# fabiojbg/LLMApiGateway

Measured on AMD Instinct MI355X. Metric: req/sec @ fixed QPS, higher is better.
Workload: dtype bf16; 1 GPU; model=llama-3-8b, global_batch=256, seq_len=192, prompt_len=128, parallelism=dp1, mode=open-loop-poisson, sampling=greedy, kv_dtype=auto

## Files before the change

### llmapigateway_amd/ops/__init__.py

```python

from __future__ import annotations

import os
from typing import Optional, Tuple

_TUNE_BASE = os.path.join(os.path.dirname(os.path.abspath(__file__)), "tunableop_gfx950.csv")
if os.path.exists(_TUNE_BASE.replace(".csv", "0.csv")):
    os.environ.setdefault("PYTORCH_TUNABLEOP_ENABLED", "1")
    os.environ.setdefault("PYTORCH_TUNABLEOP_TUNING", "0")
    os.environ.setdefault("PYTORCH_TUNABLEOP_FILENAME", _TUNE_BASE)

import torch

if torch.version.hip and os.path.exists(_TUNE_BASE.replace(".csv", "0.csv")):
    try:
        import torch.cuda.tunable as _tunable

        _tunable.enable(True)
        if os.environ.get("PYTORCH_TUNABLEOP_TUNING") != "1":
            _tunable.tuning_enable(False)
            _tunable.set_filename(_TUNE_BASE, insert_device_ordinal=True)
            _tunable.read_file(_TUNE_BASE.replace(".csv", "0.csv"))
    except Exception:
        pass

from . import reference
from .reference import build_rope_cache

_C = None
_C_ERR: Optional[str] = None
try:
    import importlib

    _C = importlib.import_module("._C", __name__)
except ImportError as e:
    _C_ERR = str(e)


def have_native() -> bool:
    return _C is not None


def _native():
    if _C is None:
        raise RuntimeError(
            "llmapigateway_amd.ops._C (gfx950 HIP extension) is not built but a GPU tensor "
            "reached the ops layer. Build it with `python setup.py build_ext --inplace` "
            f"(import error: {_C_ERR})"
        )
    return _C


def rmsnorm(x: torch.Tensor, weight: torch.Tensor, eps: float = 1e-5) -> torch.Tensor:
    if x.is_cuda:
        out = torch.empty_like(x)
        _native().rmsnorm(out, x, weight, eps)
        return out
    return reference.rmsnorm(x, weight, eps)


def rmsnorm_residual(
    x: torch.Tensor, residual: torch.Tensor, weight: torch.Tensor, eps: float = 1e-5
) -> Tuple[torch.Tensor, torch.Tensor]:
    if x.is_cuda:
        out = torch.empty_like(x)
        _native().rmsnorm_residual(out, x, residual, weight, eps)
        return out, residual
    return reference.rmsnorm_residual(x, residual, weight, eps)


def rope_inplace(
    q: torch.Tensor, k: torch.Tensor, positions: torch.Tensor, cos_sin: torch.Tensor
) -> None:
    if q.is_cuda:
        _native().rope_inplace(q, k, positions, cos_sin)
        return
    reference.rope_inplace(q, k, positions, cos_sin)


def swiglu(x: torch.Tensor) -> torch.Tensor:
    if x.is_cuda:
        inter = x.shape[-1] // 2
        out = torch.empty(
            (*x.shape[:-1], inter), dtype=x.dtype, device=x.device
        )
        _native().swiglu(out, x)
        return out
    return reference.swiglu(x)


def rope_and_kv_write(
    q: torch.Tensor,
    k: torch.Tensor,
    v: torch.Tensor,
    k_cache: torch.Tensor,
    v_cache: torch.Tensor,
    positions: torch.Tensor,
    cos_sin: torch.Tensor,
    slot_mapping: torch.Tensor,
    k_scale: Optional[torch.Tensor] = None,
    v_scale: Optional[torch.Tensor] = None,
) -> None:
    if q.is_cuda:
        _native().rope_kv_write(
            q, k, v, k_cache, v_cache, positions, cos_sin, slot_mapping,
            k_scale, v_scale,
        )
        return
    reference.rope_inplace(q, k, positions, cos_sin)
    reference.kv_cache_write(k, v, k_cache, v_cache, slot_mapping, k_scale, v_scale)


def kv_cache_write(
    k: torch.Tensor,
    v: torch.Tensor,
    k_cache: torch.Tensor,
    v_cache: torch.Tensor,
    slot_mapping: torch.Tensor,
    k_scale: Optional[torch.Tensor] = None,
    v_scale: Optional[torch.Tensor] = None,
) -> None:
    if k.is_cuda:
        _native().kv_cache_write(k, v, k_cache, v_cache, slot_mapping, k_scale, v_scale)
        return
    reference.kv_cache_write(k, v, k_cache, v_cache, slot_mapping, k_scale, v_scale)


QTILE = 64


def build_prefill_tiles(seqlens, device) -> Tuple[torch.Tensor, torch.Tensor]:
    tile_seq, tile_off = [], []
    for i, L in enumerate(seqlens):
        for off in range(0, int(L), QTILE):
            tile_seq.append(i)
            tile_off.append(off)
    return (
        torch.tensor(tile_seq, dtype=torch.int32, device=device),
        torch.tensor(tile_off, dtype=torch.int32, device=device),
    )


def attention_prefill(
    q: torch.Tensor,
    k: torch.Tensor,
    v: torch.Tensor,
    cu_seqlens: torch.Tensor,
    max_seqlen: int,
    scale: Optional[float] = None,
    causal: bool = True,
    tile_seq: Optional[torch.Tensor] = None,
    tile_off: Optional[torch.Tensor] = None,
    k_cache: Optional[torch.Tensor] = None,
    v_cache: Optional[torch.Tensor] = None,
    block_tables: Optional[torch.Tensor] = None,
    cached_lens: Optional[torch.Tensor] = None,
    k_scale: Optional[torch.Tensor] = None,
    v_scale: Optional[torch.Tensor] = None,
) -> torch.Tensor:
    if scale is None:
        scale = float(q.shape[-1]) ** -0.5
    if q.is_cuda:
        if not causal:
            raise NotImplementedError("GPU prefill kernel is causal-only")
        if tile_seq is None or tile_off is None:
            cu = cu_seqlens.cpu().tolist()
            seqlens = [cu[i + 1] - cu[i] for i in range(len(cu) - 1)]
            tile_seq, tile_off = build_prefill_tiles(seqlens, q.device)
        out = torch.empty_like(q)
        _native().attention_prefill(
            out, q, k, v, cu_seqlens.int(), tile_seq, tile_off, float(scale),
            k_cache, v_cache, block_tables, cached_lens, k_scale, v_scale,
        )
        return out
    return reference.attention_prefill(
        q, k, v, cu_seqlens, scale, causal,
        k_cache=k_cache, v_cache=v_cache,
        block_tables=block_tables, cached_lens=cached_lens,
        k_scale=k_scale, v_scale=v_scale,
    )


_SPLIT_SPAN = 2048
_DECODE_VER = int(os.environ.get("LLMAPI_DECODE_VER", "2"))
_decode_ws: dict = {}
_decode_ws_retired: list = []


def _decode_scratch(device, n_acc: int, n_ml: int):
    ws = _decode_ws.get(device.index)
    if ws is None or ws[0].numel() < n_acc or ws[1].numel() < n_ml:
        if ws is not None:
            _decode_ws_retired.append(ws)
        ws = (
            torch.empty(n_acc, dtype=torch.float32, device=device),
            torch.empty(n_ml, dtype=torch.float32, device=device),
        )
        _decode_ws[device.index] = ws
    return ws


def attention_decode(
    q: torch.Tensor,
    k_cache: torch.Tensor,
    v_cache: torch.Tensor,
    block_tables: torch.Tensor,
    context_lens: torch.Tensor,
    scale: Optional[float] = None,
    k_scale: Optional[torch.Tensor] = None,
    v_scale: Optional[torch.Tensor] = None,
) -> torch.Tensor:
    if scale is None:
        scale = float(q.shape[-1]) ** -0.5
    if q.is_cuda:
        out = torch.empty_like(q)
        B, Hq = q.shape[0], q.shape[1]
        max_ctx = block_tables.shape[1] * k_cache.shape[2]
        nsplit = 1
        if B * k_cache.shape[1] < 192 and max_ctx > _SPLIT_SPAN:
            nsplit = min(8, -(-max_ctx // _SPLIT_SPAN))
        if nsplit > 1:
            pa, pm = _decode_scratch(
                q.device, B * Hq * nsplit * q.shape[2], B * Hq * nsplit * 2
            )
            _native().attention_decode(
                out, q, k_cache, v_cache, block_tables, context_lens,
                float(scale), pa, pm, nsplit, k_scale, v_scale, 1,
            )
        else:
            _native().attention_decode(
                out, q, k_cache, v_cache, block_tables, context_lens,
                float(scale), None, None, 1, k_scale, v_scale, _DECODE_VER,
            )
        return out
    return reference.attention_decode(
        q, k_cache, v_cache, block_tables, context_lens, scale,
        k_scale=k_scale, v_scale=v_scale,
    )


_SKINNY_MAX_M = int(os.environ.get("SKINNY_GEMM_MAX_M", "16"))
_SKINNY_MAX_N = 28672
_skinny_ws: dict = {}


def _skinny_nsk(N: int, K: int) -> int:
    tiles = N // 64
    nsk = max(1, -(-256 // tiles))
    nsk = min(nsk, max(1, (K // 32) // 8), 8)
    return nsk


_skinny_ws_retired: list = []


def _skinny_scratch(device, numel: int):
    ws = _skinny_ws.get(device.index)
    if ws is None or ws.numel() < numel:
        if ws is not None:
            _skinny_ws_retired.append(ws)
        ws = torch.empty(numel, dtype=torch.float32, device=device)
        _skinny_ws[device.index] = ws
    return ws


def swizzle_weight(w: torch.Tensor) -> torch.Tensor:
    N, K = w.shape
    assert K % 32 == 0 and N % 64 == 0
    return w.view(N, K // 32, 32).permute(1, 0, 2).contiguous()


def swizzle_weight_frag(w: torch.Tensor) -> torch.Tensor:
    N, K = w.shape
    assert K % 64 == 0 and N % 64 == 0
    return (
        w.view(N // 16, 16, K // 32, 4, 8)
        .permute(2, 0, 3, 1, 4)
        .reshape(K // 32, N // 16, 64, 8)
        .contiguous()
    )


def _m256_config(M: int, N: int, K: int) -> Optional[dict]:
    if M > 256:
        return None
    if N == 8192 and K % 64 == 0 and K >= 8192:
        if K > 8192:
            return {"nf": 8, "nsk": 4, "variant": 1, "pipe": 0}
        return {"nf": 8, "nsk": 4, "variant": 0, "pipe": 0}
    if N == 7168 and K <= 8192:
        return {"nf": 4, "nsk": 3, "variant": 0, "pipe": 4}
    if N > 4096:
        return None
    if K > 8192 and N % 128 == 0:
        return {"nf": 8, "nsk": 8, "variant": 0, "pipe": 0}
    if N < 2048:
        return None
    if K < 2048:
        return {"nf": 4, "nsk": 1, "variant": 1, "pipe": 0}
    tiles = N // 64
    nsk = max(1, min(-(-256 // tiles), (K // 64) // 2, 8))
    return {"nf": 4, "nsk": nsk, "variant": 0, "pipe": 4}


def _m256_nsk(N: int, K: int, nf: int) -> int:
    tiles = N // (16 * nf)
    if tiles >= 256:
        return 1
    nsk = -(-256 // tiles)
    return max(1, min(nsk, (K // 64) // 2, 8))


_SKINNY_SWZ_MAX_M = int(os.environ.get("SKINNY_GEMM_SWZ_MAX_M", "256"))


_M256_VARIANT = int(os.environ.get("LLMAPI_M256_VARIANT", "0"))


def gemm_m256(
    x: torch.Tensor, w_frag: torch.Tensor, nf: Optional[int] = None,
    nsk: Optional[int] = None, variant: Optional[int] = None,
    pipe: Optional[int] = None,
) -> torch.Tensor:
    M, K = x.shape
    N = w_frag.shape[1] * 16
    if nf is None:
        if N % 128 == 0 and M > 64:
            nf = 8
        else:
            nf = 8 if N // 64 >= 448 else 4
    if N % (16 * nf) != 0:
        nf = 4
    if nsk is None:
        nsk = _m256_nsk(N, K, nf)
    if variant is None:
        variant = _M256_VARIANT
    if pipe is None:
        pipe = 3 if (variant == 0 and nf == 8 and K % 32 == 0) else 0
    if variant == 0:
        if pipe in (2, 3) and nf != 8:
            pipe = 0
        if pipe in (1, 4, 5) and nf != 4:
            pipe = 0
    y = torch.empty((M, N), dtype=torch.bfloat16, device=x.device)
    ws = _skinny_scratch(x.device, nsk * M * N) if nsk > 1 else None
    _native().gemm_m256(y, x, w_frag, ws, nsk, nf, variant, pipe, 0)
    return y


def _reduce_norm_covers(N: int) -> bool:
    return N % 512 == 0 and 0 < N <= 8192


def gemm_m256_rmsnorm_residual(
    x: torch.Tensor, w_frag: torch.Tensor, residual: torch.Tensor,
    norm_w: torch.Tensor, eps: float, nf: int, nsk: int, variant: int = 0,
    pipe: int = 0,
) -> Tuple[torch.Tensor, torch.Tensor]:
    M, K = x.shape
    N = w_frag.shape[1] * 16
    if nsk < 2:
        raise ValueError("fused reduce+norm needs split-K slabs (nsk > 1)")
    out = torch.empty((M, N), dtype=torch.bfloat16, device=x.device)
    ws = _skinny_scratch(x.device, nsk * M * N)
    _native().gemm_m256(
        out, x, w_frag, ws, nsk, nf, variant, pipe, 0,
        residual, norm_w, float(eps), out,
    )
    return out, residual


def _m256_route(
    x: torch.Tensor, w: torch.Tensor, w_swz: Optional[torch.Tensor]
) -> Optional[dict]:
    M = x.shape[0]
    if not (
        x.is_cuda
        and x.dim() == 2
        and x.dtype == torch.bfloat16
        and w.dtype == torch.bfloat16
        and w.shape[0] % 64 == 0
        and w.shape[0] <= _SKINNY_MAX_N
        and w.shape[1] % 64 == 0
        and x.is_contiguous()
        and w.is_contiguous()
        and w_swz is not None
        and w_swz.dim() == 4
        and 8 < M <= 256
    ):
        return None
    return _m256_config(M, w.shape[0], w.shape[1])


def linear_rmsnorm_residual(
    x: torch.Tensor, w: torch.Tensor, w_swz: Optional[torch.Tensor],
    residual: torch.Tensor, norm_w: torch.Tensor, eps: float = 1e-5,
) -> Tuple[torch.Tensor, torch.Tensor]:
    if not x.is_cuda:
        return reference.linear_rmsnorm_residual(x, w, residual, norm_w, eps)
    if not os.environ.get("LLMAPI_NO_DECODE_FUSION"):
        cfg = _m256_route(x, w, w_swz)
        if (
            cfg is not None
            and cfg["nsk"] > 1
            and _reduce_norm_covers(w.shape[0])
            and residual.is_contiguous()
        ):
            return gemm_m256_rmsnorm_residual(
                x, w_swz, residual, norm_w, eps, **cfg
            )
    return rmsnorm_residual(linear(x, w, w_swz), residual, norm_w, eps)


def interleave_gate_up(w: torch.Tensor) -> torch.Tensor:
    two_i, K = w.shape
    assert two_i % 32 == 0
    return w.view(2, two_i // 32, 16, K).transpose(0, 1).reshape(two_i, K)


def gemm_m256_swiglu(
    x: torch.Tensor, w_frag: torch.Tensor, nf: int = 8, variant: int = 1,
    pipe: int = 0,
) -> torch.Tensor:
    M, K = x.shape
    N = w_frag.shape[1] * 16
    y = torch.empty((M, N // 2), dtype=torch.bfloat16, device=x.device)
    _native().gemm_m256(y, x, w_frag, None, 1, nf, variant, pipe, 1)
    return y


def _m256_swiglu_config(M: int, N: int, K: int) -> Optional[dict]:
    if os.environ.get("LLMAPI_NO_FUSED_SWIGLU"):
        return None
    if not (8 < M <= 256):
        return None
    if N == 28672 and K == 4096:
        if M <= 128:
            return {"nf": 8, "variant": 0, "pipe": 0}
        return {"nf": 8, "variant": 1, "pipe": 0}
    if N == 7168 and K == 4096:
        return {"nf": 4, "variant": 0, "pipe": 4}
    return None


def swiglu_linear(
    x: torch.Tensor, w: torch.Tensor,
    w_swz: Optional[torch.Tensor] = None,
    w_int: Optional[torch.Tensor] = None,
) -> torch.Tensor:
    if w_int is not None and x.dim() == 2:
        cfg = _m256_swiglu_config(x.shape[0], w_int.shape[1] * 16, x.shape[1])
        if cfg is not None:
            return gemm_m256_swiglu(x, w_int, **cfg)
    return swiglu(linear(x, w, w_swz))


def linear(
    x: torch.Tensor, w: torch.Tensor, w_swz: Optional[torch.Tensor] = None
) -> torch.Tensor:
    M = x.shape[0]
    if (
        x.is_cuda
        and x.dtype == torch.bfloat16
        and w.dtype == torch.bfloat16
        and 0 < M
        and w.shape[0] % 64 == 0
        and w.shape[0] <= _SKINNY_MAX_N
        and w.shape[1] % 32 == 0
        and x.is_contiguous()
        and w.is_contiguous()
    ):
        N, K = w.shape
        if (
            w_swz is not None
            and w_swz.dim() == 4
            and 8 < M <= 256
            and K % 64 == 0
        ):
            cfg = _m256_config(M, N, K)
            if cfg is not None:
                return gemm_m256(x, w_swz, **cfg)
            return torch.nn.functional.linear(x, w)
        if w_swz is not None and w_swz.dim() == 3 and M <= _SKINNY_SWZ_MAX_M:
            y = torch.empty((M, N), dtype=torch.bfloat16, device=x.device)
            nsk = _skinny_nsk(N, K)
            ws = _skinny_scratch(x.device, nsk * M * N) if nsk > 1 else None
            _native().gemm_skinny(y, x, w_swz, ws, nsk, True)
            return y
        if M <= _SKINNY_MAX_M:
            y = torch.empty((M, N), dtype=torch.bfloat16, device=x.device)
            nsk = _skinny_nsk(N, K)
            ws = _skinny_scratch(x.device, nsk * M * N) if nsk > 1 else None
            _native().gemm_skinny(y, x, w, ws, nsk, False)
            return y
    return torch.nn.functional.linear(x, w)


def topk_topp_filter(
    logits: torch.Tensor, topp: torch.Tensor, topk: torch.Tensor
) -> torch.Tensor:
    if logits.is_cuda:
        _native().topk_topp_filter(logits, topp, topk)
        return logits
    return reference.topk_topp_filter(logits, topp, topk)


def sample(
    logits: torch.Tensor,
    temperature: torch.Tensor,
    noise: Optional[torch.Tensor] = None,
) -> torch.Tensor:
    if logits.is_cuda:
        out = torch.empty(logits.shape[0], dtype=torch.long, device=logits.device)
        _native().sample(out, logits, temperature, noise)
        return out
    return reference.sample(logits, temperature, noise)


__all__ = [
    "have_native",
    "build_rope_cache",
    "rmsnorm",
    "rmsnorm_residual",
    "rope_inplace",
    "rope_and_kv_write",
    "swiglu",
    "kv_cache_write",
    "linear",
    "gemm_m256",
    "gemm_m256_rmsnorm_residual",
    "linear_rmsnorm_residual",
    "swizzle_weight",
    "swizzle_weight_frag",
    "attention_prefill",
    "attention_decode",
    "sample",
    "topk_topp_filter",
    "reference",
]
```

### llmapigateway_amd/ops/csrc/attention_decode.hip

```cpp

#include "common.h"

#define MAX_G 8
#define NWAVES 4
#define DECODE_D 128
#define SPLIT_SPAN 2048

template <int G, bool SPLIT, bool FP8>
__launch_bounds__(NWAVES* WAVE_SIZE)
__global__ void attention_decode_kernel(
    bf16* __restrict__ out,
    const bf16* __restrict__ q,
    const void* __restrict__ k_cache,
    const void* __restrict__ v_cache,
    const float* __restrict__ k_scale,
    const float* __restrict__ v_scale,
    const int* __restrict__ block_tables,
    const int* __restrict__ context_lens,
    float scale,
    int Hq,
    int Hkv,
    int block_size,
    int max_blocks,
    int64_t q_stride,
    float* __restrict__ part_acc,
    float* __restrict__ part_ml,
    int nsplit) {
    const int seq = blockIdx.x;
    const int kvh = blockIdx.y;
    const int split = SPLIT ? blockIdx.z : 0;
    const int D = DECODE_D;
    const int L = context_lens[seq];
    if (L <= 0) return;
    const int span0 = SPLIT ? split * SPLIT_SPAN : 0;
    if (SPLIT && span0 >= L) {
        const int lane0 = threadIdx.x & (WAVE_SIZE - 1);
        if (threadIdx.x < WAVE_SIZE) {
#pragma unroll
            for (int g = 0; g < G; ++g) {
                const size_t pb =
                    (((size_t)seq * Hq + kvh * G + g) * nsplit + split);
                if (lane0 < 2) part_ml[pb * 2 + lane0] = lane0 == 0 ? -INFINITY : 0.f;
                for (int d = lane0; d < D; d += WAVE_SIZE) part_acc[pb * D + d] = 0.f;
            }
        }
        return;
    }
    const int span1 = SPLIT ? min(L, span0 + SPLIT_SPAN) : L;

    const int tid = threadIdx.x;
    const int lane = tid & (WAVE_SIZE - 1);
    const int wave = tid >> 6;

    __shared__ float q_lds[G][DECODE_D];
    __shared__ float p_lds[NWAVES][G][WAVE_SIZE];
    __shared__ float m_lds[NWAVES][G];
    __shared__ float l_lds[NWAVES][G];
    __shared__ float acc_lds[NWAVES][G][DECODE_D];
    __shared__ int bt_lds[1024];

    for (int i = tid; i < G * D; i += blockDim.x) {
        const int g = i / D, d = i % D;
        q_lds[g][d] =
            bf2f(q[(size_t)seq * q_stride + (size_t)(kvh * G + g) * D + d]) * scale;
    }
    const int nblocks = (L + block_size - 1) / block_size;
    for (int i = tid; i < nblocks && i < 1024; i += blockDim.x)
        bt_lds[i] = block_tables[(size_t)seq * max_blocks + i];
    __syncthreads();
    const int* __restrict__ bt_global = block_tables + (size_t)seq * max_blocks;
#define BT(idx) ((idx) < 1024 ? bt_lds[(idx)] : bt_global[(idx)])

    float m[G], l[G], acc[G][4];
#pragma unroll
    for (int g = 0; g < G; ++g) {
        m[g] = -INFINITY;
        l[g] = 0.f;
#pragma unroll
        for (int d = 0; d < 4; ++d) acc[g][d] = 0.f;
    }

    const int c0 = span0 / WAVE_SIZE;
    const int nchunks = (span1 + WAVE_SIZE - 1) / WAVE_SIZE;
    for (int c = c0 + wave; c < nchunks; c += NWAVES) {
        const int pos = c * WAVE_SIZE + lane;
        const bool valid = pos < span1;

        float s[G];
#pragma unroll
        for (int g = 0; g < G; ++g) s[g] = valid ? 0.f : -INFINITY;
        if (valid) {
            const int kblock = BT(pos / block_size);
            const int koff = pos % block_size;
            const size_t krow_i = ((size_t)kblock * Hkv + kvh) * block_size + koff;
#pragma unroll 4
            for (int i = 0; i < D / 8; ++i) {
                float kf[8];
                if (FP8) {
                    const uint2 kq = reinterpret_cast<const uint2*>(
                        (const unsigned char*)k_cache + krow_i * D)[i];
                    fp8x4_to_f32(kq.x, kf[0], kf[1], kf[2], kf[3]);
                    fp8x4_to_f32(kq.y, kf[4], kf[5], kf[6], kf[7]);
                } else {
                    const uint4 kv8 = reinterpret_cast<const uint4*>(
                        (const bf16*)k_cache + krow_i * D)[i];
                    unpack2(kv8.x, kf[0], kf[1]);
                    unpack2(kv8.y, kf[2], kf[3]);
                    unpack2(kv8.z, kf[4], kf[5]);
                    unpack2(kv8.w, kf[6], kf[7]);
                }
#pragma unroll
                for (int g = 0; g < G; ++g) {
                    const float4 qa = *reinterpret_cast<const float4*>(&q_lds[g][i * 8]);
                    const float4 qb = *reinterpret_cast<const float4*>(&q_lds[g][i * 8 + 4]);
                    s[g] = fmaf(qa.x, kf[0], s[g]);
                    s[g] = fmaf(qa.y, kf[1], s[g]);
                    s[g] = fmaf(qa.z, kf[2], s[g]);
                    s[g] = fmaf(qa.w, kf[3], s[g]);
                    s[g] = fmaf(qb.x, kf[4], s[g]);
                    s[g] = fmaf(qb.y, kf[5], s[g]);
                    s[g] = fmaf(qb.z, kf[6], s[g]);
                    s[g] = fmaf(qb.w, kf[7], s[g]);
                }
            }
            if (FP8) {
                const float ksc = k_scale[krow_i];
#pragma unroll
                for (int g = 0; g < G; ++g) s[g] *= ksc;
            }
        }

#pragma unroll
        for (int g = 0; g < G; ++g) {
            const float cmax = wave_reduce_max(s[g]);
            const float m_new = fmaxf(m[g], cmax);
            float p = 0.f;
            if (valid && m_new != -INFINITY) p = __expf(s[g] - m_new);
            const float factor = (m[g] == -INFINITY) ? 0.f : __expf(m[g] - m_new);
            const float csum = wave_reduce_sum(p);
            l[g] = l[g] * factor + csum;
#pragma unroll
            for (int d = 0; d < 4; ++d) acc[g][d] *= factor;
            m[g] = m_new;
            p_lds[wave][g][lane] = p;
        }

        const int dbase = (lane & 31) * 4;
        const int khalf = lane >> 5;
#pragma unroll 2
        for (int j = 0; j < WAVE_SIZE; j += 8) {
            uint2 vp[4];
            uint32_t vp8[4];
            float vsc[4];
#pragma unroll
            for (int u = 0; u < 4; ++u) {
                const int pos = min(c * WAVE_SIZE + j + 2 * u + khalf, span1 - 1);
                const int vb = BT(pos / block_size);
                const int vo = pos % block_size;
                const size_t vrow_i = ((size_t)vb * Hkv + kvh) * block_size + vo;
                if (FP8) {
                    vp8[u] = *reinterpret_cast<const uint32_t*>(
                        (const unsigned char*)v_cache + vrow_i * D + dbase);
                    vsc[u] = v_scale[vrow_i];
                } else {
                    vp[u] = *reinterpret_cast<const uint2*>(
                        (const bf16*)v_cache + vrow_i * D + dbase);
                }
            }
#pragma unroll
            for (int u = 0; u < 4; ++u) {
                float v0, v1, v2, v3;
                if (FP8) {
                    fp8x4_to_f32(vp8[u], v0, v1, v2, v3);
                } else {
                    unpack2(vp[u].x, v0, v1);
                    unpack2(vp[u].y, v2, v3);
                }
                const int key = j + 2 * u + khalf;
#pragma unroll
                for (int g = 0; g < G; ++g) {
                    const float pj = p_lds[wave][g][key] * (FP8 ? vsc[u] : 1.f);
                    acc[g][0] = fmaf(pj, v0, acc[g][0]);
                    acc[g][1] = fmaf(pj, v1, acc[g][1]);
                    acc[g][2] = fmaf(pj, v2, acc[g][2]);
                    acc[g][3] = fmaf(pj, v3, acc[g][3]);
                }
            }
        }
    }

#pragma unroll
    for (int g = 0; g < G; ++g)
#pragma unroll
        for (int d = 0; d < 4; ++d) acc[g][d] += __shfl_xor(acc[g][d], 32, WAVE_SIZE);

#pragma unroll
    for (int g = 0; g < G; ++g) {
        if (lane == 0) {
            m_lds[wave][g] = m[g];
            l_lds[wave][g] = l[g];
        }
        if (lane < 32) {
#pragma unroll
            for (int d = 0; d < 4; ++d)
                acc_lds[wave][g][(lane & 31) * 4 + d] = acc[g][d];
        }
    }
    __syncthreads();

    if (wave == 0) {
#pragma unroll
        for (int g = 0; g < G; ++g) {
            float gm = -INFINITY;
#pragma unroll
            for (int w = 0; w < NWAVES; ++w) gm = fmaxf(gm, m_lds[w][g]);
            float gl = 0.f;
            float f[NWAVES];
#pragma unroll
            for (int w = 0; w < NWAVES; ++w) {
                f[w] = (m_lds[w][g] == -INFINITY) ? 0.f : __expf(m_lds[w][g] - gm);
                gl += f[w] * l_lds[w][g];
            }
            float o0 = 0.f, o1 = 0.f;
#pragma unroll
            for (int w = 0; w < NWAVES; ++w) {
                o0 += f[w] * acc_lds[w][g][2 * lane];
                o1 += f[w] * acc_lds[w][g][2 * lane + 1];
            }
            if (SPLIT) {
                const size_t pb =
                    (((size_t)seq * Hq + kvh * G + g) * nsplit + split);
                part_acc[pb * DECODE_D + 2 * lane] = o0;
                part_acc[pb * DECODE_D + 2 * lane + 1] = o1;
                if (lane == 0) {
                    part_ml[pb * 2] = gm;
                    part_ml[pb * 2 + 1] = gl;
                }
            } else {
                const float inv_l = (gl > 0.f) ? 1.f / gl : 0.f;
                reinterpret_cast<uint32_t*>(
                    out + (size_t)seq * Hq * DECODE_D +
                    (size_t)(kvh * G + g) * DECODE_D)[lane] =
                    pack2(o0 * inv_l, o1 * inv_l);
            }
        }
    }
}

typedef __attribute__((__vector_size__(8 * sizeof(short)))) short bf16x8_d;


template <int G, bool SPLIT, bool FP8>
__launch_bounds__(NWAVES* WAVE_SIZE)
__global__ void attention_decode_v2_kernel(
    bf16* __restrict__ out,
    const bf16* __restrict__ q,
    const void* __restrict__ k_cache,
    const void* __restrict__ v_cache,
    const float* __restrict__ k_scale,
    const float* __restrict__ v_scale,
    const int* __restrict__ block_tables,
    const int* __restrict__ context_lens,
    float scale,
    int Hq,
    int Hkv,
    int block_size,
    int max_blocks,
    int64_t q_stride,
    float* __restrict__ part_acc,
    float* __restrict__ part_ml,
    int nsplit) {
    const int seq = blockIdx.x;
    const int kvh = blockIdx.y;
    const int split = SPLIT ? blockIdx.z : 0;
    const int D = DECODE_D;
    const int L = context_lens[seq];
    if (L <= 0) return;
    const int span0 = SPLIT ? split * SPLIT_SPAN : 0;
    const int tid = threadIdx.x;
    const int lane = tid & (WAVE_SIZE - 1);
    const int wave = tid >> 6;
    constexpr int HPW = (G + NWAVES - 1) / NWAVES;
    if (SPLIT && span0 >= L) {
#pragma unroll
        for (int hh = 0; hh < HPW; ++hh) {
            const int g = wave + hh * NWAVES;
            if (g >= G) break;
            const size_t pb = (((size_t)seq * Hq + kvh * G + g) * nsplit + split);
            if (lane < 2) part_ml[pb * 2 + lane] = lane == 0 ? -INFINITY : 0.f;
            for (int d = lane; d < D; d += WAVE_SIZE) part_acc[pb * D + d] = 0.f;
        }
        return;
    }
    const int span1 = SPLIT ? min(L, span0 + SPLIT_SPAN) : L;

    __shared__ float q_lds[G][DECODE_D];
    __shared__ bf16 k_lds[WAVE_SIZE][DECODE_D];
    __shared__ bf16 v_lds[WAVE_SIZE][DECODE_D];
    __shared__ float p_lds[G][WAVE_SIZE];
    __shared__ int bt_lds[1024];

    for (int i = tid; i < G * D; i += blockDim.x) {
        const int g = i / D, d = i % D;
        q_lds[g][d] =
            bf2f(q[(size_t)seq * q_stride + (size_t)(kvh * G + g) * D + d]) * scale;
    }
    const int nblocks = (L + block_size - 1) / block_size;
    for (int i = tid; i < nblocks && i < 1024; i += blockDim.x)
        bt_lds[i] = block_tables[(size_t)seq * max_blocks + i];
    __syncthreads();
    const int* __restrict__ bt_global = block_tables + (size_t)seq * max_blocks;
#define BT2(idx) ((idx) < 1024 ? bt_lds[(idx)] : bt_global[(idx)])

    float m[HPW], l[HPW], acc[HPW][4];
#pragma unroll
    for (int h = 0; h < HPW; ++h) {
        m[h] = -INFINITY;
        l[h] = 0.f;
#pragma unroll
        for (int d = 0; d < 4; ++d) acc[h][d] = 0.f;
    }

    const int c0 = span0 / WAVE_SIZE;
    const int nchunks = (span1 + WAVE_SIZE - 1) / WAVE_SIZE;
    for (int c = c0; c < nchunks; ++c) {
        __syncthreads();
        for (int pass = 0; pass < 4; ++pass) {
            const int key = (pass << 4) | (tid >> 4);
            const int chunk = tid & 15;
            const int pos = c * WAVE_SIZE + key;
            const int cpos = min(pos, span1 - 1);
            const int blk = BT2(cpos / block_size);
            const size_t row =
                ((size_t)blk * Hkv + kvh) * block_size + cpos % block_size;
            const int kchunk = chunk ^ (key & 15);
            if (FP8) {
                const uint2 kq = reinterpret_cast<const uint2*>(
                    (const unsigned char*)k_cache + row * D)[chunk];
                const uint2 vq = reinterpret_cast<const uint2*>(
                    (const unsigned char*)v_cache + row * D)[chunk];
                const float ksc = k_scale[row], vsc = v_scale[row];
                float kf[8], vf[8];
                fp8x4_to_f32(kq.x, kf[0], kf[1], kf[2], kf[3]);
                fp8x4_to_f32(kq.y, kf[4], kf[5], kf[6], kf[7]);
                fp8x4_to_f32(vq.x, vf[0], vf[1], vf[2], vf[3]);
                fp8x4_to_f32(vq.y, vf[4], vf[5], vf[6], vf[7]);
                uint2 kw, vw;
                kw.x = pack2_trunc(kf[0] * ksc, kf[1] * ksc);
                kw.y = pack2_trunc(kf[2] * ksc, kf[3] * ksc);
                uint2 kw2;
                kw2.x = pack2_trunc(kf[4] * ksc, kf[5] * ksc);
                kw2.y = pack2_trunc(kf[6] * ksc, kf[7] * ksc);
                vw.x = pack2_trunc(vf[0] * vsc, vf[1] * vsc);
                vw.y = pack2_trunc(vf[2] * vsc, vf[3] * vsc);
                uint2 vw2;
                vw2.x = pack2_trunc(vf[4] * vsc, vf[5] * vsc);
                vw2.y = pack2_trunc(vf[6] * vsc, vf[7] * vsc);
                uint4 kq4 = {kw.x, kw.y, kw2.x, kw2.y};
                uint4 vq4 = {vw.x, vw.y, vw2.x, vw2.y};
                *reinterpret_cast<uint4*>(&k_lds[key][kchunk * 8]) = kq4;
                *reinterpret_cast<uint4*>(&v_lds[key][chunk * 8]) = vq4;
            } else {
                *reinterpret_cast<uint4*>(&k_lds[key][kchunk * 8]) =
                    reinterpret_cast<const uint4*>((const bf16*)k_cache + row * D)[chunk];
                *reinterpret_cast<uint4*>(&v_lds[key][chunk * 8]) =
                    reinterpret_cast<const uint4*>((const bf16*)v_cache + row * D)[chunk];
            }
        }
        __syncthreads();

        const int pos = c * WAVE_SIZE + lane;
        const bool valid = pos < span1;
#pragma unroll
        for (int hh = 0; hh < HPW; ++hh) {
            const int g = wave + hh * NWAVES;
            if (g >= G) break;
            float sg = valid ? 0.f : -INFINITY;
            if (valid) {
#pragma unroll 4
                for (int i = 0; i < D / 8; ++i) {
                    const bf16x8_d kv8 = *reinterpret_cast<const bf16x8_d*>(
                        &k_lds[lane][(i ^ (lane & 15)) * 8]);
                    const uint4 kvu = *reinterpret_cast<const uint4*>(&kv8);
                    float kf[8];
                    unpack2(kvu.x, kf[0], kf[1]);
                    unpack2(kvu.y, kf[2], kf[3]);
                    unpack2(kvu.z, kf[4], kf[5]);
                    unpack2(kvu.w, kf[6], kf[7]);
                    const float4 qa = *reinterpret_cast<const float4*>(&q_lds[g][i * 8]);
                    const float4 qb = *reinterpret_cast<const float4*>(&q_lds[g][i * 8 + 4]);
                    sg = fmaf(qa.x, kf[0], sg);
                    sg = fmaf(qa.y, kf[1], sg);
                    sg = fmaf(qa.z, kf[2], sg);
                    sg = fmaf(qa.w, kf[3], sg);
                    sg = fmaf(qb.x, kf[4], sg);
                    sg = fmaf(qb.y, kf[5], sg);
                    sg = fmaf(qb.z, kf[6], sg);
                    sg = fmaf(qb.w, kf[7], sg);
                }
            }
            const float cmax = wave_reduce_max(sg);
            const float m_new = fmaxf(m[hh], cmax);
            float pv = 0.f;
            if (valid && m_new != -INFINITY) pv = __expf(sg - m_new);
            const float factor = (m[hh] == -INFINITY) ? 0.f : __expf(m[hh] - m_new);
            const float csum = wave_reduce_sum(pv);
            l[hh] = l[hh] * factor + csum;
#pragma unroll
            for (int d = 0; d < 4; ++d) acc[hh][d] *= factor;
            m[hh] = m_new;
            p_lds[g][lane] = pv;
        }

        const int dbase = (lane & 31) * 4;
        const int khalf = lane >> 5;
#pragma unroll
        for (int hh = 0; hh < HPW; ++hh) {
            const int g = wave + hh * NWAVES;
            if (g >= G) break;
#pragma unroll 4
            for (int j = 0; j < WAVE_SIZE; j += 2) {
                const int key = j + khalf;
                const float pj = p_lds[g][key];
                float v0, v1, v2, v3;
                const uint2 vv = *reinterpret_cast<const uint2*>(&v_lds[key][dbase]);
                unpack2(vv.x, v0, v1);
                unpack2(vv.y, v2, v3);
                acc[hh][0] = fmaf(pj, v0, acc[hh][0]);
                acc[hh][1] = fmaf(pj, v1, acc[hh][1]);
                acc[hh][2] = fmaf(pj, v2, acc[hh][2]);
                acc[hh][3] = fmaf(pj, v3, acc[hh][3]);
            }
        }
    }

#pragma unroll
    for (int hh = 0; hh < HPW; ++hh) {
        const int g = wave + hh * NWAVES;
        if (g >= G) break;
#pragma unroll
        for (int d = 0; d < 4; ++d) acc[hh][d] += __shfl_xor(acc[hh][d], 32, WAVE_SIZE);
        if (lane < 32) {
            if (SPLIT) {
                const size_t pb = (((size_t)seq * Hq + kvh * G + g) * nsplit + split);
#pragma unroll
                for (int d = 0; d < 4; ++d)
                    part_acc[pb * DECODE_D + (lane & 31) * 4 + d] = acc[hh][d];
                if (lane == 0) {
                    part_ml[pb * 2] = m[hh];
                    part_ml[pb * 2 + 1] = l[hh];
                }
            } else {
                const float inv_l = (l[hh] > 0.f) ? 1.f / l[hh] : 0.f;
                uint2 o2;
                o2.x = pack2(acc[hh][0] * inv_l, acc[hh][1] * inv_l);
                o2.y = pack2(acc[hh][2] * inv_l, acc[hh][3] * inv_l);
                *reinterpret_cast<uint2*>(
                    out + (size_t)seq * Hq * DECODE_D +
                    (size_t)(kvh * G + g) * DECODE_D + (lane & 31) * 4) = o2;
            }
        }
    }
}

template <int G, bool SPLIT, bool FP8>
__launch_bounds__(NWAVES* WAVE_SIZE)
__global__ void attention_decode_v3_kernel(
    bf16* __restrict__ out,
    const bf16* __restrict__ q,
    const void* __restrict__ k_cache,
    const void* __restrict__ v_cache,
    const float* __restrict__ k_scale,
    const float* __restrict__ v_scale,
    const int* __restrict__ block_tables,
    const int* __restrict__ context_lens,
    float scale,
    int Hq,
    int Hkv,
    int block_size,
    int max_blocks,
    int64_t q_stride,
    float* __restrict__ part_acc,
    float* __restrict__ part_ml,
    int nsplit) {
    const int seq = blockIdx.x;
    const int kvh = blockIdx.y;
    const int split = SPLIT ? blockIdx.z : 0;
    const int D = DECODE_D;
    const int L = context_lens[seq];
    if (L <= 0) return;
    const int span0 = SPLIT ? split * SPLIT_SPAN : 0;
    const int tid = threadIdx.x;
    const int lane = tid & (WAVE_SIZE - 1);
    const int wave = tid >> 6;
    constexpr int HPW = (G + NWAVES - 1) / NWAVES;
    if (SPLIT && span0 >= L) {
#pragma unroll
        for (int hh = 0; hh < HPW; ++hh) {
            const int g = wave + hh * NWAVES;
            if (g >= G) break;
            const size_t pb = (((size_t)seq * Hq + kvh * G + g) * nsplit + split);
            if (lane < 2) part_ml[pb * 2 + lane] = lane == 0 ? -INFINITY : 0.f;
            for (int d = lane; d < D; d += WAVE_SIZE) part_acc[pb * D + d] = 0.f;
        }
        return;
    }
    const int span1 = SPLIT ? min(L, span0 + SPLIT_SPAN) : L;

    __shared__ float q_lds[G][DECODE_D];
    __shared__ bf16 k_lds[WAVE_SIZE][DECODE_D];
    __shared__ float p_lds[G][WAVE_SIZE];
    __shared__ int bt_lds[1024];

    for (int i = tid; i < G * D; i += blockDim.x) {
        const int g = i / D, d = i % D;
        q_lds[g][d] =
            bf2f(q[(size_t)seq * q_stride + (size_t)(kvh * G + g) * D + d]) * scale;
    }
    const int nblocks = (L + block_size - 1) / block_size;
    for (int i = tid; i < nblocks && i < 1024; i += blockDim.x)
        bt_lds[i] = block_tables[(size_t)seq * max_blocks + i];
    __syncthreads();
    const int* __restrict__ bt_global = block_tables + (size_t)seq * max_blocks;
#define BT2(idx) ((idx) < 1024 ? bt_lds[(idx)] : bt_global[(idx)])

    float m[HPW], l[HPW], acc[HPW][4];
#pragma unroll
    for (int h = 0; h < HPW; ++h) {
        m[h] = -INFINITY;
        l[h] = 0.f;
#pragma unroll
        for (int d = 0; d < 4; ++d) acc[h][d] = 0.f;
    }

    const int c0 = span0 / WAVE_SIZE;
    const int nchunks = (span1 + WAVE_SIZE - 1) / WAVE_SIZE;
    for (int c = c0; c < nchunks; ++c) {
        __syncthreads();
        for (int pass = 0; pass < 4; ++pass) {
            const int key = (pass << 4) | (tid >> 4);
            const int chunk = tid & 15;
            const int pos = c * WAVE_SIZE + key;
            const int cpos = min(pos, span1 - 1);
            const int blk = BT2(cpos / block_size);
            const size_t row =
                ((size_t)blk * Hkv + kvh) * block_size + cpos % block_size;
            const int kchunk = chunk ^ (key & 15);
            if (FP8) {
                const uint2 kq = reinterpret_cast<const uint2*>(
                    (const unsigned char*)k_cache + row * D)[chunk];
                const float ksc = k_scale[row];
                float kf[8];
                fp8x4_to_f32(kq.x, kf[0], kf[1], kf[2], kf[3]);
                fp8x4_to_f32(kq.y, kf[4], kf[5], kf[6], kf[7]);
                uint4 kq4;
                kq4.x = pack2_trunc(kf[0] * ksc, kf[1] * ksc);
                kq4.y = pack2_trunc(kf[2] * ksc, kf[3] * ksc);
                kq4.z = pack2_trunc(kf[4] * ksc, kf[5] * ksc);
                kq4.w = pack2_trunc(kf[6] * ksc, kf[7] * ksc);
                *reinterpret_cast<uint4*>(&k_lds[key][kchunk * 8]) = kq4;
            } else {
                *reinterpret_cast<uint4*>(&k_lds[key][kchunk * 8]) =
                    reinterpret_cast<const uint4*>((const bf16*)k_cache + row * D)[chunk];
            }
        }
        __syncthreads();

        const int pos = c * WAVE_SIZE + lane;
        const bool valid = pos < span1;
#pragma unroll
        for (int hh = 0; hh < HPW; ++hh) {
            const int g = wave + hh * NWAVES;
            if (g >= G) break;
            float sg = valid ? 0.f : -INFINITY;
            if (valid) {
#pragma unroll 4
                for (int i = 0; i < D / 8; ++i) {
                    const bf16x8_d kv8 = *reinterpret_cast<const bf16x8_d*>(
                        &k_lds[lane][(i ^ (lane & 15)) * 8]);
                    const uint4 kvu = *reinterpret_cast<const uint4*>(&kv8);
                    float kf[8];
                    unpack2(kvu.x, kf[0], kf[1]);
                    unpack2(kvu.y, kf[2], kf[3]);
                    unpack2(kvu.z, kf[4], kf[5]);
                    unpack2(kvu.w, kf[6], kf[7]);
                    const float4 qa = *reinterpret_cast<const float4*>(&q_lds[g][i * 8]);
                    const float4 qb = *reinterpret_cast<const float4*>(&q_lds[g][i * 8 + 4]);
                    sg = fmaf(qa.x, kf[0], sg);
                    sg = fmaf(qa.y, kf[1], sg);
                    sg = fmaf(qa.z, kf[2], sg);
                    sg = fmaf(qa.w, kf[3], sg);
                    sg = fmaf(qb.x, kf[4], sg);
                    sg = fmaf(qb.y, kf[5], sg);
                    sg = fmaf(qb.z, kf[6], sg);
                    sg = fmaf(qb.w, kf[7], sg);
                }
            }
            const float cmax = wave_reduce_max(sg);
            const float m_new = fmaxf(m[hh], cmax);
            float pv = 0.f;
            if (valid && m_new != -INFINITY) pv = __expf(sg - m_new);
            const float factor = (m[hh] == -INFINITY) ? 0.f : __expf(m[hh] - m_new);
            const float csum = wave_reduce_sum(pv);
            l[hh] = l[hh] * factor + csum;
#pragma unroll
            for (int d = 0; d < 4; ++d) acc[hh][d] *= factor;
            m[hh] = m_new;
            p_lds[g][lane] = pv;
        }

        const int dbase = (lane & 31) * 4;
        const int khalf = lane >> 5;
#pragma unroll 2
        for (int j = 0; j < WAVE_SIZE; j += 8) {
            uint2 vp[4];
            uint32_t vp8[4];
            float vsc4[4];
#pragma unroll
            for (int u = 0; u < 4; ++u) {
                const int pos2 = min(c * WAVE_SIZE + j + 2 * u + khalf, span1 - 1);
                const int vb = BT2(pos2 / block_size);
                const int vo = pos2 % block_size;
                const size_t vrow = ((size_t)vb * Hkv + kvh) * block_size + vo;
                if (FP8) {
                    vp8[u] = *reinterpret_cast<const uint32_t*>(
                        (const unsigned char*)v_cache + vrow * D + dbase);
                    vsc4[u] = v_scale[vrow];
                } else {
                    vp[u] = *reinterpret_cast<const uint2*>(
                        (const bf16*)v_cache + vrow * D + dbase);
                }
            }
#pragma unroll
            for (int u = 0; u < 4; ++u) {
                float v0, v1, v2, v3;
                if (FP8) {
                    fp8x4_to_f32(vp8[u], v0, v1, v2, v3);
                } else {
                    unpack2(vp[u].x, v0, v1);
                    unpack2(vp[u].y, v2, v3);
                }
                const int key = j + 2 * u + khalf;
#pragma unroll
                for (int hh = 0; hh < HPW; ++hh) {
                    const int g = wave + hh * NWAVES;
                    if (g >= G) break;
                    const float pj = p_lds[g][key] * (FP8 ? vsc4[u] : 1.f);
                    acc[hh][0] = fmaf(pj, v0, acc[hh][0]);
                    acc[hh][1] = fmaf(pj, v1, acc[hh][1]);
                    acc[hh][2] = fmaf(pj, v2, acc[hh][2]);
                    acc[hh][3] = fmaf(pj, v3, acc[hh][3]);
                }
            }
        }
    }

#pragma unroll
    for (int hh = 0; hh < HPW; ++hh) {
        const int g = wave + hh * NWAVES;
        if (g >= G) break;
#pragma unroll
        for (int d = 0; d < 4; ++d) acc[hh][d] += __shfl_xor(acc[hh][d], 32, WAVE_SIZE);
        if (lane < 32) {
            if (SPLIT) {
                const size_t pb = (((size_t)seq * Hq + kvh * G + g) * nsplit + split);
#pragma unroll
                for (int d = 0; d < 4; ++d)
                    part_acc[pb * DECODE_D + (lane & 31) * 4 + d] = acc[hh][d];
                if (lane == 0) {
                    part_ml[pb * 2] = m[hh];
                    part_ml[pb * 2 + 1] = l[hh];
                }
            } else {
                const float inv_l = (l[hh] > 0.f) ? 1.f / l[hh] : 0.f;
                uint2 o2;
                o2.x = pack2(acc[hh][0] * inv_l, acc[hh][1] * inv_l);
                o2.y = pack2(acc[hh][2] * inv_l, acc[hh][3] * inv_l);
                *reinterpret_cast<uint2*>(
                    out + (size_t)seq * Hq * DECODE_D +
                    (size_t)(kvh * G + g) * DECODE_D + (lane & 31) * 4) = o2;
            }
        }
    }
}


__global__ void decode_combine_kernel(
    bf16* __restrict__ out,
    const float* __restrict__ part_acc,
    const float* __restrict__ part_ml,
    int nsplit) {
    const int bh = blockIdx.x;
    const int lane = threadIdx.x;
    const size_t base = (size_t)bh * nsplit;
    float gm = -INFINITY;
    for (int z = 0; z < nsplit; ++z) gm = fmaxf(gm, part_ml[(base + z) * 2]);
    float gl = 0.f, o0 = 0.f, o1 = 0.f;
    for (int z = 0; z < nsplit; ++z) {
        const float mz = part_ml[(base + z) * 2];
        const float f = (mz == -INFINITY) ? 0.f : __expf(mz - gm);
        gl += f * part_ml[(base + z) * 2 + 1];
        o0 += f * part_acc[(base + z) * DECODE_D + 2 * lane];
        o1 += f * part_acc[(base + z) * DECODE_D + 2 * lane + 1];
    }
    const float inv_l = (gl > 0.f) ? 1.f / gl : 0.f;
    reinterpret_cast<uint32_t*>(out + (size_t)bh * DECODE_D)[lane] =
        pack2(o0 * inv_l, o1 * inv_l);
}

extern "C" hipError_t launch_attention_decode(
    void* out, const void* q, const void* k_cache, const void* v_cache,
    const float* k_scale, const float* v_scale,
    const int* block_tables, const int* context_lens, float scale, int B,
    int Hq, int Hkv, int block_size, int max_blocks, int D, int64_t q_stride,
    float* part_acc, float* part_ml, int nsplit, int version,
    hipStream_t stream) {
    if (D != DECODE_D) return hipErrorNotSupported;
    if (Hq % Hkv != 0) return hipErrorInvalidValue;
    if (nsplit > 1 && (part_acc == nullptr || part_ml == nullptr))
        return hipErrorInvalidValue;
    const int G = Hq / Hkv;
    const bool fp8 = k_scale != nullptr;
    dim3 grid(B, Hkv, nsplit > 1 ? nsplit : 1);
    dim3 block(NWAVES * WAVE_SIZE);
#define LAUNCH_G3(GV, SPLIT, FP8V)                                             \
    do {                                                                       \
        if (version == 2)                                                      \
            attention_decode_v2_kernel<GV, SPLIT, FP8V>                        \
                <<<grid, block, 0, stream>>>(                                  \
                    (bf16*)out, (const bf16*)q, k_cache, v_cache, k_scale,     \
                    v_scale, block_tables, context_lens, scale, Hq, Hkv,       \
                    block_size, max_blocks, q_stride, part_acc, part_ml,       \
                    nsplit);                                                   \
        else                                                                   \
            attention_decode_kernel<GV, SPLIT, FP8V>                           \
                <<<grid, block, 0, stream>>>(                                  \
                    (bf16*)out, (const bf16*)q, k_cache, v_cache, k_scale,     \
                    v_scale, block_tables, context_lens, scale, Hq, Hkv,       \
                    block_size, max_blocks, q_stride, part_acc, part_ml,       \
                    nsplit);                                                   \
    } while (0)
#define LAUNCH_G2(GV, SPLIT)                                                   \
    do {                                                                       \
        if (fp8) LAUNCH_G3(GV, SPLIT, true); else LAUNCH_G3(GV, SPLIT, false);\
    } while (0)
#define LAUNCH_G(GV)                                                           \
    do {                                                                       \
        if (nsplit > 1) LAUNCH_G2(GV, true); else LAUNCH_G2(GV, false);        \
    } while (0)
    switch (G) {
        case 1: LAUNCH_G(1); break;
        case 2: LAUNCH_G(2); break;
        case 3: LAUNCH_G(3); break;
        case 4: LAUNCH_G(4); break;
        case 5: LAUNCH_G(5); break;
        case 6: LAUNCH_G(6); break;
        case 7: LAUNCH_G(7); break;
        case 8: LAUNCH_G(8); break;
        default: return hipErrorInvalidValue;
    }
#undef LAUNCH_G
#undef LAUNCH_G2
#undef LAUNCH_G3
    if (nsplit > 1) {
        decode_combine_kernel<<<dim3(B * Hq), dim3(WAVE_SIZE), 0, stream>>>(
            (bf16*)out, part_acc, part_ml, nsplit);
    }
    HIP_CHECK_LAST();
    return hipSuccess;
}
```

Baseline: 189.9 req/s.

## Add register-prefetched decode attention kernel staging K and V through LDS

Adds a v4 decode attention kernel and makes it the default instead of v2. Each iteration prefetches the next chunk's K and V rows into registers while the current chunk is being computed. V is now staged in LDS with coalesced loads, replacing strided per-lane global reads. The Q load is issued before the early-exit check, and PV accumulation is bounded to the valid keys. The costs are more registers, an extra LDS buffer for V, and a new code path that may lower occupancy.

Result: no change. 189.3 req/s (-0.3%).

```diff
diff --git a/llmapigateway_amd/ops/__init__.py b/llmapigateway_amd/ops/__init__.py
--- a/llmapigateway_amd/ops/__init__.py
+++ b/llmapigateway_amd/ops/__init__.py
@@ -182,7 +182,7 @@
 
 
 _SPLIT_SPAN = 2048
-_DECODE_VER = int(os.environ.get("LLMAPI_DECODE_VER", "2"))
+_DECODE_VER = int(os.environ.get("LLMAPI_DECODE_VER", "4"))
 _decode_ws: dict = {}
 _decode_ws_retired: list = []
 
diff --git a/llmapigateway_amd/ops/csrc/attention_decode.hip b/llmapigateway_amd/ops/csrc/attention_decode.hip
--- a/llmapigateway_amd/ops/csrc/attention_decode.hip
+++ b/llmapigateway_amd/ops/csrc/attention_decode.hip
@@ -463,9 +463,102 @@
     }
 }
 
+
+template <bool FP8>
+struct DecodeStage;
+template <>
+struct DecodeStage<false> {
+    uint4 k[4], v[4];
+};
+template <>
+struct DecodeStage<true> {
+    uint2 k[4], v[4];
+    float ks[4], vs[4];
+};
+
+template <bool FP8, typename BTF>
+__device__ __forceinline__ void decode_stage_load(
+    DecodeStage<FP8>& st, int c, int span1, int tid, int Hkv, int kvh,
+    int block_size, const void* __restrict__ k_cache,
+    const void* __restrict__ v_cache, const float* __restrict__ k_scale,
+    const float* __restrict__ v_scale, BTF bt) {
+    const int D = DECODE_D;
+    const int chunk = tid & 15;
+    int blk[4];
+#pragma unroll
+    for (int pass = 0; pass < 4; ++pass) {
+        const int pos = c * WAVE_SIZE + ((pass << 4) | (tid >> 4));
+        blk[pass] = bt(min(pos, span1 - 1) / block_size);
+    }
+    asm volatile("" ::"v"(blk[0]), "v"(blk[1]), "v"(blk[2]), "v"(blk[3]));
+#pragma unroll
+    for (int pass = 0; pass < 4; ++pass) {
+        const int pos = c * WAVE_SIZE + ((pass << 4) | (tid >> 4));
+        const size_t row =
+            ((size_t)blk[pass] * Hkv + kvh) * block_size + pos % block_size;
+        if constexpr (FP8) {
+            st.k[pass] = make_uint2(0u, 0u);
+            st.v[pass] = make_uint2(0u, 0u);
+            st.ks[pass] = 0.f;
+            st.vs[pass] = 0.f;
+            if (pos < span1) {
+                st.k[pass] = reinterpret_cast<const uint2*>(
+                    (const unsigned char*)k_cache + row * D)[chunk];
+                st.v[pass] = reinterpret_cast<const uint2*>(
+                    (const unsigned char*)v_cache + row * D)[chunk];
+                st.ks[pass] = k_scale[row];
+                st.vs[pass] = v_scale[row];
+            }
+        } else {
+            st.k[pass] = make_uint4(0u, 0u, 0u, 0u);
+            st.v[pass] = make_uint4(0u, 0u, 0u, 0u);
+            if (pos < span1) {
+                st.k[pass] = reinterpret_cast<const uint4*>(
+                    (const bf16*)k_cache + row * D)[chunk];
+                st.v[pass] = reinterpret_cast<const uint4*>(
+                    (const bf16*)v_cache + row * D)[chunk];
+            }
+        }
+    }
+}
+
+template <bool FP8>
+__device__ __forceinline__ void decode_stage_write(
+    const DecodeStage<FP8>& st, int tid, bf16 (*k_lds)[DECODE_D],
+    bf16 (*v_lds)[DECODE_D]) {
+    const int chunk = tid & 15;
+#pragma unroll
+    for (int pass = 0; pass < 4; ++pass) {
+        const int key = (pass << 4) | (tid >> 4);
+        const int kchunk = chunk ^ (key & 15);
+        if constexpr (FP8) {
+            const float ksc = st.ks[pass], vsc = st.vs[pass];
+            float kf[8], vf[8];
+            fp8x4_to_f32(st.k[pass].x, kf[0], kf[1], kf[2], kf[3]);
+            fp8x4_to_f32(st.k[pass].y, kf[4], kf[5], kf[6], kf[7]);
+            fp8x4_to_f32(st.v[pass].x, vf[0], vf[1], vf[2], vf[3]);
+            fp8x4_to_f32(st.v[pass].y, vf[4], vf[5], vf[6], vf[7]);
+            uint4 kq4, vq4;
+            kq4.x = pack2_trunc(kf[0] * ksc, kf[1] * ksc);
+            kq4.y = pack2_trunc(kf[2] * ksc, kf[3] * ksc);
+            kq4.z = pack2_trunc(kf[4] * ksc, kf[5] * ksc);
+            kq4.w = pack2_trunc(kf[6] * ksc, kf[7] * ksc);
+            vq4.x = pack2_trunc(vf[0] * vsc, vf[1] * vsc);
+            vq4.y = pack2_trunc(vf[2] * vsc, vf[3] * vsc);
+            vq4.z = pack2_trunc(vf[4] * vsc, vf[5] * vsc);
+            vq4.w = pack2_trunc(vf[6] * vsc, vf[7] * vsc);
+            *reinterpret_cast<uint4*>(&k_lds[key][kchunk * 8]) = kq4;
+            *reinterpret_cast<uint4*>(&v_lds[key][chunk * 8]) = vq4;
+        } else {
+            *reinterpret_cast<uint4*>(&k_lds[key][kchunk * 8]) = st.k[pass];
+            *reinterpret_cast<uint4*>(&v_lds[key][chunk * 8]) = st.v[pass];
+        }
+    }
+}
+
 template <int G, bool SPLIT, bool FP8>
 __launch_bounds__(NWAVES* WAVE_SIZE)
-__global__ void attention_decode_v3_kernel(
+__global__ void attention_decode_v4_kernel(
     bf16* __restrict__ out,
     const bf16* __restrict__ q,
     const void* __restrict__ k_cache,
@@ -487,10 +580,17 @@
     const int kvh = blockIdx.y;
     const int split = SPLIT ? blockIdx.z : 0;
     const int D = DECODE_D;
+    const int tid = threadIdx.x;
+    constexpr int QN = (G * DECODE_D + NWAVES * WAVE_SIZE - 1) / (NWAVES * WAVE_SIZE);
+    bf16 qv[QN];
+#pragma unroll
+    for (int u = 0; u < QN; ++u) {
+        const int i = min(tid + u * NWAVES * WAVE_SIZE, G * D - 1);
+        qv[u] = q[(size_t)seq * q_stride + (size_t)(kvh * G) * D + i];
+    }
     const int L = context_lens[seq];
     if (L <= 0) return;
     const int span0 = SPLIT ? split * SPLIT_SPAN : 0;
-    const int tid = threadIdx.x;
     const int lane = tid & (WAVE_SIZE - 1);
     const int wave = tid >> 6;
     constexpr int HPW = (G + NWAVES - 1) / NWAVES;
@@ -509,20 +609,30 @@
 
     __shared__ float q_lds[G][DECODE_D];
     __shared__ bf16 k_lds[WAVE_SIZE][DECODE_D];
+    __shared__ bf16 v_lds[WAVE_SIZE][DECODE_D];
     __shared__ float p_lds[G][WAVE_SIZE];
     __shared__ int bt_lds[1024];
 
-    for (int i = tid; i < G * D; i += blockDim.x) {
-        const int g = i / D, d = i % D;
-        q_lds[g][d] =
-            bf2f(q[(size_t)seq * q_stride + (size_t)(kvh * G + g) * D + d]) * scale;
-    }
+    const int c0 = span0 / WAVE_SIZE;
+    const int nchunks = (span1 + WAVE_SIZE - 1) / WAVE_SIZE;
+    const int* __restrict__ bt_global = block_tables + (size_t)seq * max_blocks;
+
     const int nblocks = (L + block_size - 1) / block_size;
-    for (int i = tid; i < nblocks && i < 1024; i += blockDim.x)
-        bt_lds[i] = block_tables[(size_t)seq * max_blocks + i];
-    __syncthreads();
-    const int* __restrict__ bt_global = block_tables + (size_t)seq * max_blocks;
-#define BT2(idx) ((idx) < 1024 ? bt_lds[(idx)] : bt_global[(idx)])
+    const int bt_first = bt_global[min(tid, nblocks - 1)];
+    DecodeStage<FP8> st;
+    decode_stage_load<FP8>(st, c0, span1, tid, Hkv, kvh, block_size, k_cache,
+                           v_cache, k_scale, v_scale,
+                           [&](int idx) { return bt_global[idx]; });
+
+#pragma unroll
+    for (int u = 0; u < QN; ++u) {
+        const int i = tid + u * NWAVES * WAVE_SIZE;
+        if (i < G * D) q_lds[i / D][i % D] = bf2f(qv[u]) * scale;
+    }
+    if (tid < nblocks) bt_lds[tid] = bt_first;
+    for (int i = tid + NWAVES * WAVE_SIZE; i < nblocks && i < 1024;
+         i += NWAVES * WAVE_SIZE)
+        bt_lds[i] = bt_global[i];
 
     float m[HPW], l[HPW], acc[HPW][4];
 #pragma unroll
@@ -533,38 +643,22 @@
         for (int d = 0; d < 4; ++d) acc[h][d] = 0.f;
     }
 
-    const int c0 = span0 / WAVE_SIZE;
-    const int nchunks = (span1 + WAVE_SIZE - 1) / WAVE_SIZE;
     for (int c = c0; c < nchunks; ++c) {
+        if (c != c0) __syncthreads();
+        decode_stage_write<FP8>(st, tid, k_lds, v_lds);
         __syncthreads();
-        for (int pass = 0; pass < 4; ++pass) {
-            const int key = (pass << 4) | (tid >> 4);
-            const int chunk = tid & 15;
-            const int pos = c * WAVE_SIZE + key;
-            const int cpos = min(pos, span1 - 1);
-            const int blk = BT2(cpos / block_size);
-            const size_t row =
-                ((size_t)blk * Hkv + kvh) * block_size + cpos % block_size;
-            const int kchunk = chunk ^ (key & 15);
-            if (FP8) {
-                const uint2 kq = reinterpret_cast<const uint2*>(
-                    (const unsigned char*)k_cache + row * D)[chunk];
-                const float ksc = k_scale[row];
-                float kf[8];
-                fp8x4_to_f32(kq.x, kf[0], kf[1], kf[2], kf[3]);
-                fp8x4_to_f32(kq.y, kf[4], kf[5], kf[6], kf[7]);
-                uint4 kq4;
-                kq4.x = pack2_trunc(kf[0] * ksc, kf[1] * ksc);
-                kq4.y = pack2_trunc(kf[2] * ksc, kf[3] * ksc);
-                kq4.z = pack2_trunc(kf[4] * ksc, kf[5] * ksc);
-                kq4.w = pack2_trunc(kf[6] * ksc, kf[7] * ksc);
-                *reinterpret_cast<uint4*>(&k_lds[key][kchunk * 8]) = kq4;
-            } else {
-                *reinterpret_cast<uint4*>(&k_lds[key][kchunk * 8]) =
-                    reinterpret_cast<const uint4*>((const bf16*)k_cache + row * D)[chunk];
-            }
-        }
-        __syncthreads();
+        if (c + 1 < nchunks) {
+            if (((c + 1) * WAVE_SIZE + WAVE_SIZE - 1) / block_size < 1024)
+                decode_stage_load<FP8>(
+                    st, c + 1, span1, tid, Hkv, kvh, block_size, k_cache,
+                    v_cache, k_scale, v_scale,
+                    [&](int idx) { return bt_lds[idx]; });
+            else
+                decode_stage_load<FP8>(
+                    st, c + 1, span1, tid, Hkv, kvh, block_size, k_cache,
+                    v_cache, k_scale, v_scale,
+                    [&](int idx) { return bt_global[idx]; });
+        }
 
         const int pos = c * WAVE_SIZE + lane;
         const bool valid = pos < span1;
@@ -611,41 +705,20 @@
 
         const int dbase = (lane & 31) * 4;
         const int khalf = lane >> 5;
-#pragma unroll 2
-        for (int j = 0; j < WAVE_SIZE; j += 8) {
-            uint2 vp[4];
-            uint32_t vp8[4];
-            float vsc4[4];
-#pragma unroll
-            for (int u = 0; u < 4; ++u) {
-                const int pos2 = min(c * WAVE_SIZE + j + 2 * u + khalf, span1 - 1);
-                const int vb = BT2(pos2 / block_size);
-                const int vo = pos2 % block_size;
-                const size_t vrow = ((size_t)vb * Hkv + kvh) * block_size + vo;
-                if (FP8) {
-                    vp8[u] = *reinterpret_cast<const uint32_t*>(
-                        (const unsigned char*)v_cache + vrow * D + dbase);
-                    vsc4[u] = v_scale[vrow];
-                } else {
-                    vp[u] = *reinterpret_cast<const uint2*>(
-                        (const bf16*)v_cache + vrow * D + dbase);
-                }
-            }
-#pragma unroll
-            for (int u = 0; u < 4; ++u) {
-                float v0, v1, v2, v3;
-                if (FP8) {
-                    fp8x4_to_f32(vp8[u], v0, v1, v2, v3);
-                } else {
-                    unpack2(vp[u].x, v0, v1);
-                    unpack2(vp[u].y, v2, v3);
-                }
-                const int key = j + 2 * u + khalf;
-#pragma unroll
-                for (int hh = 0; hh < HPW; ++hh) {
-                    const int g = wave + hh * NWAVES;
-                    if (g >= G) break;
-                    const float pj = p_lds[g][key] * (FP8 ? vsc4[u] : 1.f);
+        const int jend = min(WAVE_SIZE, (span1 - c * WAVE_SIZE + 7) & ~7);
+#pragma unroll
+        for (int hh = 0; hh < HPW; ++hh) {
+            const int g = wave + hh * NWAVES;
+            if (g >= G) break;
+            for (int j0 = 0; j0 < jend; j0 += 8) {
+#pragma unroll
+                for (int j = j0; j < j0 + 8; j += 2) {
+                    const int key = j + khalf;
+                    const float pj = p_lds[g][key];
+                    float v0, v1, v2, v3;
+                    const uint2 vv = *reinterpret_cast<const uint2*>(&v_lds[key][dbase]);
+                    unpack2(vv.x, v0, v1);
+                    unpack2(vv.y, v2, v3);
                     acc[hh][0] = fmaf(pj, v0, acc[hh][0]);
                     acc[hh][1] = fmaf(pj, v1, acc[hh][1]);
                     acc[hh][2] = fmaf(pj, v2, acc[hh][2]);
@@ -725,7 +798,14 @@
     dim3 block(NWAVES * WAVE_SIZE);
 #define LAUNCH_G3(GV, SPLIT, FP8V)                                             \
     do {                                                                       \
-        if (version == 2)                                                      \
+        if (version == 4)                                                      \
+            attention_decode_v4_kernel<GV, SPLIT, FP8V>                        \
+                <<<grid, block, 0, stream>>>(                                  \
+                    (bf16*)out, (const bf16*)q, k_cache, v_cache, k_scale,     \
+                    v_scale, block_tables, context_lens, scale, Hq, Hkv,       \
+                    block_size, max_blocks, q_stride, part_acc, part_ml,       \
+                    nsplit);                                                   \
+        else if (version == 2)                                                 \
             attention_decode_v2_kernel<GV, SPLIT, FP8V>                        \
                 <<<grid, block, 0, stream>>>(                                  \
                     (bf16*)out, (const bf16*)q, k_cache, v_cache, k_scale,     \
```
